# ebu/libear

Hardware: AMD Instinct MI355X
Metric: Msamples/s (higher is better)
Workload: dtype f32 io / f16x2-split MFMA, f32 accumulate

## Files before the change

libear_amd/csrc/api_render.hip:

```cpp
#include <cmath>
#include <cstdlib>
#include <chrono>
#include <memory>
#include <vector>

#include "common.h"
#include "curves.h"
#include "host_pipeline.h"
#include "pcm_frames.h"
#include "fft_kernels.h"
#include "render_kernels.h"

using namespace earhip;

namespace earhip {
std::vector<cf> make_twiddles(int L) {
  std::vector<cf> tw(L);
  const double pi = 3.14159265358979323846264338327950288;
  for (int t = 0; t < L; t++) {
    const double a = -2.0 * pi * (double)t / (double)L;
    tw[t] = cf_make((float)std::cos(a), (float)std::sin(a));
  }
  return tw;
}

template <int L>
static void launch_spectrum_t(const float *in, size_t stride, int n_valid, const cf *tw, cf *out,
                              int rows, hipStream_t s) {
  hipLaunchKernelGGL((k_spectrum_real<L>), dim3(rows), dim3(kFftThreads), 0, s, in, stride,
                     n_valid, tw, out);
}
void launch_spectrum(int L, const float *in, size_t stride, int n_valid, const cf *tw, cf *out,
                     int rows, hipStream_t s) {
  switch (L) {
    case 64: launch_spectrum_t<64>(in, stride, n_valid, tw, out, rows, s); break;
    case 128: launch_spectrum_t<128>(in, stride, n_valid, tw, out, rows, s); break;
    case 256: launch_spectrum_t<256>(in, stride, n_valid, tw, out, rows, s); break;
    case 512: launch_spectrum_t<512>(in, stride, n_valid, tw, out, rows, s); break;
    case 1024: launch_spectrum_t<1024>(in, stride, n_valid, tw, out, rows, s); break;
    case 2048: launch_spectrum_t<2048>(in, stride, n_valid, tw, out, rows, s); break;
    case 4096: launch_spectrum_t<4096>(in, stride, n_valid, tw, out, rows, s); break;
    case 8192: launch_spectrum_t<8192>(in, stride, n_valid, tw, out, rows, s); break;
    default: {
      FftShape S;
      if (!fft_make_shape(L, &S)) fail_invalid("FFT size must be in [4, 8192]");
      hipLaunchKernelGGL(k_spectrum_real_rt, dim3(rows), dim3(kFftThreads), fft_rt_lds(k_spectrum_real_rt, L), s, S,
                         in, stride, n_valid, tw, out);
    }
  }
  EARHIP_HIP(hipGetLastError());
}
}

template <int L>
static void launch_decor_t(const DecorParams &P, dim3 grid, hipStream_t s) {
  hipLaunchKernelGGL((k_decorrelate_delay_mix<L>), grid, dim3(256), 0, s, P);
}
static void launch_decor(int L, const DecorParams &P, dim3 grid, hipStream_t s, bool force_wg) {
  switch (L) {
    case 128: launch_decor_t<128>(P, grid, s); break;
    case 256: launch_decor_t<256>(P, grid, s); break;
    case 512: launch_decor_t<512>(P, grid, s); break;
    case 1024:
      if (force_wg) {
        launch_decor_t<1024>(P, grid, s);
      } else {
        hipLaunchKernelGGL(k_decorrelate_wave, dim3((grid.x + kDecorWaves - 1) / kDecorWaves, grid.y),
                           dim3(64 * kDecorWaves), 0, s, P);
      }
      break;
    case 2048: launch_decor_t<2048>(P, grid, s); break;
    case 4096: launch_decor_t<4096>(P, grid, s); break;
    case 8192: launch_decor_t<8192>(P, grid, s); break;
    default: {
      FftShape S;
      if (!fft_make_shape(L, &S)) fail_invalid("block_size must be in [16, 4096]");
      const size_t lds = fft_rt_lds(k_decorrelate_delay_mix_rt, L, sizeof(float) * (L / 2));
      hipLaunchKernelGGL(k_decorrelate_delay_mix_rt, grid, dim3(256), lds, s, P, S);
    }
  }
  EARHIP_HIP(hipGetLastError());
}

static int wave_run_len(int T, int N, int num_cus) {
  const double c[4] = {0.0, 6.9, 9.3, 12.2};
  int best = 1;
  double best_cost = 1e30;
  for (int R = 1; R <= 31; R += 2) {
    const long runs = (T + R - 1) / R;
    const long wgs = (runs + earhip::kDecorWaves - 1) / earhip::kDecorWaves * N;
    const long full = wgs / (3L * num_cus), rem = wgs - full * 3L * num_cus;
    const double pairs = (R + 1) / 2;
    const double cost = pairs * (full * c[3] + c[(rem + num_cus - 1) / num_cus]);
    if (cost <= best_cost) best_cost = cost, best = R;
    if (runs == 1) break;
  }
  return best;
}

struct earhip_render {
  earhip_ctx *ctx = nullptr;
  int M = 0, N = 0, B = 0, K = 1, D = 0, T = 0;
  int Bk = 0, Lk = 0;
  int NP = 1;
  std::unique_ptr<CurveSet> curves;
  int64_t t = 0;
  int last_plan[3] = {0, 0, 0};
  int last_paired = -1;
  size_t last_scratch_bytes = 0;
  long scratch_regrows = 0;
  DevBuf<unsigned> rec;
  bool last_gated = false;
  bool last_device_form = false;
  bool last_hg_robust = false;
  int last_kind = -1;
  int run_len = 11;
  bool run_len_set = false;

  DevBuf<SegDesc> desc;
  DevBuf<float> bus;
  int max_gsplit = 1;
  DevBuf<cf> H, tw;
  DevBuf<float> tail[2], dly[2], hist[2];
  DevBuf<float> ztail, zdly, zhist;
  bool fresh = true;
  int cur = 0;
  DevBuf<float> d_in, d_out;
  PinBuf<float> p_in, p_out;
  std::unique_ptr<GatherPool> gather;
  StreamPipe pipe;
  int last_host_chunks = 0;
  PinBuf<unsigned char> p_bytes;
  DevBuf<unsigned char> d_bytes;
  DevBuf<float> d_ilv, d_rows, d_rows_out;
  DevBuf<unsigned char> d_pcm;
  PinBuf<unsigned char> p_pcm;
  PcmLevels levels;
  bool timing = false;
  bool last_timed = false;
  int timing_every = 1;
  long timing_calls = 0;
  hipEvent_t ev[6] = {nullptr, nullptr, nullptr, nullptr, nullptr, nullptr};
  struct Pending { hipEvent_t e[6]; bool has_k2; bool continues; };
  std::vector<Pending> pending;
  std::vector<hipEvent_t> pool;
  double acc_ms[3] = {0, 0, 0};
  double acc_n[3] = {0, 0, 0};

  ~earhip_render() {
    for (auto &p : pending)
      for (auto e : p.e)
        if (e) (void)hipEventDestroy(e);
    for (auto e : pool) (void)hipEventDestroy(e);
  }

  unsigned mode_word() {
    ctx->use();
    unsigned word = 0;
    EARHIP_HIP(hipMemcpyAsync(&word, rec.p, sizeof(word), hipMemcpyDeviceToHost, ctx->stream));
    EARHIP_HIP(hipStreamSynchronize(ctx->stream));
    if (!(word & kModeRecorded)) fail_internal("no gain kernel recorded the call's mode word");
    return word;
  }

  hipEvent_t get_event() {
    if (!pool.empty()) {
      hipEvent_t e = pool.back();
      pool.pop_back();
      return e;
    }
    hipEvent_t e;
    EARHIP_HIP(hipEventCreate(&e));
    return e;
  }

  void drain_timing() {
    EARHIP_HIP(hipStreamSynchronize(ctx->stream));
    for (auto &p : pending) {
      float ms = 0;
      const double one = p.continues ? 0.0 : 1.0;
      EARHIP_HIP(hipEventElapsedTime(&ms, p.e[0], p.e[1]));
      acc_ms[2] += ms; acc_n[2] += one;
      EARHIP_HIP(hipEventElapsedTime(&ms, p.e[2], p.e[3]));
      acc_ms[0] += ms; acc_n[0] += one;
      if (p.has_k2) {
        EARHIP_HIP(hipEventElapsedTime(&ms, p.e[4], p.e[5]));
        acc_ms[1] += ms; acc_n[1] += one;
      }
      for (auto e : p.e)
        if (e) pool.push_back(e);
    }
    pending.clear();
  }

  size_t direct_stride(const float *const *ch, int count, size_t n) const {
    if (ctx->host_ranges.empty() || count < 1) return 0;
    const uintptr_t a0 = (uintptr_t)ch[0];
    const uintptr_t step = count > 1 ? (uintptr_t)ch[1] - a0 : sizeof(float) * n;
    if ((a0 & 15) != 0 || step % 16 != 0 || step < sizeof(float) * n || step > ((uintptr_t)1 << 40)) return 0;
    for (int c = 1; c < count; c++)
      if ((uintptr_t)ch[c] - (uintptr_t)ch[c - 1] != step) return 0;
    return ctx->host_reachable(ch[0], step * (count - 1) + sizeof(float) * n) ? (size_t)(step / sizeof(float)) : 0;
  }

  size_t frames_to_device_rows(size_t nblocks, const void *frames_dev, int fmt, int frame_channels, int first_channel, bool with_out) {
    ctx->use();
    const size_t S = (size_t)pcm_sample_bytes(fmt), n = nblocks * (size_t)B, cap = (size_t)T * B;
    if (d_rows.n < cap * M || (with_out && d_rows_out.n < cap * N)) {
      EARHIP_HIP(hipStreamSynchronize(ctx->stream));
      d_rows.reserve(cap * M);
      if (with_out) d_rows_out.reserve(cap * N);
    }
    launch_pcm_to_rows(fmt, frames_dev, (size_t)frame_channels * S, (size_t)first_channel * S, M, n, d_rows.p, n, ctx->stream);
    return n;
  }
  void reserve_pcm_out(size_t bytes, bool pinned) {
    levels.reserve(N, ctx->stream);
    d_pcm.reserve(bytes);
    if (pinned) p_pcm.reserve(bytes);
  }

  HostChunkPlan host_plan(size_t nblocks, bool direct) const {
    return plan_host_chunks(nblocks, B, M, direct, ctx->has(OPT_HOST_CHUNK_MB), ctx->get(OPT_HOST_CHUNK_MB), ctx->get(OPT_HOST_FIRST, 0));
  }
  hipError_t chunk_rows_d2h(float *out0, size_t out_st, size_t at, size_t len) {
    const float *dout = d_out.p + (size_t)N * at;
    if (out_st)
      return hipMemcpy2DAsync(out0 + at, sizeof(float) * out_st, dout, sizeof(float) * len, sizeof(float) * len, N, hipMemcpyDeviceToHost, pipe.out);
    return hipMemcpyAsync(p_out.p + (size_t)N * at, dout, sizeof(float) * len * N, hipMemcpyDeviceToHost, pipe.out);
  }
  void chunk_rows_scatter(float *const *out, size_t at, size_t len) const {
    for (int ch = 0; ch < N; ch++) std::memcpy(out[ch] + at, p_out.p + (size_t)N * at + (size_t)ch * len, sizeof(float) * len);
  }
  void process_short_call(size_t nblocks, float *out0, size_t out_st) {
    const size_t n = nblocks * (size_t)B;
    const bool direct_out = NP <= 1;
    process_device(nblocks, d_in.p, n, out_st ? out0 : direct_out ? p_out.p : d_out.p, out_st ? out_st : n);
    if (!out_st && !direct_out) EARHIP_HIP(hipMemcpyAsync(p_out.p, d_out.p, sizeof(float) * n * N, hipMemcpyDeviceToHost, ctx->stream));
  }
  GatherPool &staging_threads() {
    if (!gather) {
      gather.reset(new GatherPool);
      const int want = ctx->get(OPT_HOST_THREADS, 0);
      gather->start(want >= 1 && want <= 64 ? want : default_staging_threads());
    }
    return *gather;
  }

  MixLaunch plan_call(size_t nblocks, size_t in_stride) {
    const int nsamples = (int)(nblocks * (size_t)B);
    MixLaunch ml = plan_mix(ctx, curves->plan(), M, nsamples, ctx->strict, max_gsplit, curves->aligned_tile(t),
                            curves->ramp_share(), curves->gain_scale(), curves->point_density_all(), curves->pair_waste(256), curves->pair_waste(512),
                            curves->hinge_exact_share(in_stride, (size_t)nsamples), curves->tiles_aligned(kF32GridTile, t),
                            curves->deltas_per_pair(256));
    const size_t bus_stride = ((size_t)nsamples + 3) & ~(size_t)3;
    while (ml.gsplit > 1 && bus_stride * K * N * ml.gsplit > bus.n) ml.gsplit /= 2;
    return ml;
  }

  size_t last_in_stride = 0;
  void reserve_for_curves() {
    size_t need = 0;
    bool hinge = false;
    const size_t lens[3] = {(size_t)T, (size_t)std::max(1, T / 2), (size_t)1};
    for (size_t nb : lens) {
      const MixLaunch ml = plan_call(nb, last_in_stride ? last_in_stride : nb * (size_t)B);
      need = std::max(need, scratch_units(*curves, ml, M));
      hinge = hinge || ml.hinge;
    }
    if (hinge) curves->ensure_kinks(ctx);
// ... 3 lines not shown
    }
  }

  int resident_workgroups(const MixLaunch &ml) const {
    if (!(ml.split || ml.pieces || ml.hinge)) return 0;
    return ctx->num_cus * (ml.tile() >= 512 ? 1 : 2);
  }

  struct BusTap {
    float *sink = nullptr;
    size_t stride = 0, cap = 0, pos = 0;
    void attach(bool on, float *sink_dev, size_t sink_stride, size_t sink_capacity) {
      if (on) {
        require(sink_dev != nullptr, "sink_dev must not be NULL");
        require(sink_stride >= sink_capacity, "sink_stride must be >= sink_capacity");
      }
      *this = on ? BusTap{sink_dev, sink_stride, sink_capacity, 0} : BusTap{};
    }
  };
  earhip_loudness *meter = nullptr;
  earhip_firmix *fm = nullptr;
  earhip_limiter *lim = nullptr;
  BusTap fm_tap, lim_tap;
  void check_taps(size_t nblocks) const {
    const size_t n = nblocks * (size_t)B;
    if (meter) loudness_check_room(meter, n);
    if (fm) {
      firmix_check_room(fm, nblocks);
      if (fm_tap.pos + n > fm_tap.cap) fail_invalid("the call would pass the FIR matrix's sink_capacity (nothing was rendered)");
    }
    if (lim) {
      limiter_check_room(lim, n);
      if (lim_tap.pos + n > lim_tap.cap) fail_invalid("the call would pass the limiter's sink_capacity (nothing was rendered)");
    }
  }
  void feed_taps(size_t nblocks, const float *out_dev, size_t out_stride) {
    const size_t n = nblocks * (size_t)B;
    if (meter) loudness_feed(meter, n, out_dev, out_stride);
    if (fm) {
      firmix_feed(fm, nblocks, out_dev, out_stride, fm_tap.sink + fm_tap.pos, fm_tap.stride);
      fm_tap.pos += n;
    }
    if (lim) {
      limiter_feed(lim, n, out_dev, out_stride, lim_tap.sink + lim_tap.pos, lim_tap.stride);
      lim_tap.pos += n;
    }
  }
  void process_device(size_t nblocks, const float *in_dev, size_t in_stride, float *out_dev, size_t out_stride) {
    if (!meter && !fm && !lim) return render_spans(nblocks, in_dev, in_stride, out_dev, out_stride);
    check_taps(nblocks);
    render_spans(nblocks, in_dev, in_stride, out_dev, out_stride);
    feed_taps(nblocks, out_dev, out_stride);
  }
  void render_spans(size_t nblocks, const float *in_dev, size_t in_stride, float *out_dev, size_t out_stride) {
    MixLaunch whole;
    bool have_plan = false;
    if (!ctx->strict && ctx->get(OPT_TAILCUT, 1) != 0 && nblocks >= 2) {
      last_in_stride = in_stride;
      if (curves->dirty()) {
        curves->commit(ctx);
        reserve_for_curves();
      }
      const MixLaunch ml = whole = plan_call(nblocks, in_stride);
      have_plan = true;
      const int W = resident_workgroups(ml);
      if (W > 0 && ml.gsplit == 1 && ml.ntiles > W) {
        const size_t tile = (size_t)ml.tile();
        const size_t full = (size_t)ml.ntiles / (size_t)W, rest = (size_t)ml.ntiles % (size_t)W;
        const size_t main_samples = full * (size_t)W * tile;
        const size_t eighths = (size_t)std::min(std::max(ctx->get(OPT_TAILCUT, 2), 0), 7);
        if (rest > 0 && rest <= (size_t)W * eighths / 8 && main_samples % (size_t)B == 0) {
          const size_t main_blocks = main_samples / (size_t)B;
          process_span(main_blocks, in_dev, in_stride, out_dev, out_stride, false);
          const int kind = last_kind, plan3[3] = {last_plan[0], last_plan[1], last_plan[2]};
          const size_t scratch = last_scratch_bytes;
          const bool gated = last_gated, device_form = last_device_form, hg_robust = last_hg_robust;
          const int paired = last_paired;
          process_span(nblocks - main_blocks, in_dev + main_samples, in_stride, out_dev + main_samples, out_stride, true);
          last_kind = kind;
          last_gated = gated, last_device_form = device_form, last_paired = paired, last_hg_robust = hg_robust;
          for (int i = 0; i < 3; i++) last_plan[i] = plan3[i];
          last_scratch_bytes = scratch;
          last_tail_blocks = (int)(nblocks - main_blocks);
          return;
        }
      }
    }
    last_tail_blocks = 0;
    process_span(nblocks, in_dev, in_stride, out_dev, out_stride, false, have_plan ? &whole : nullptr);
  }
  int last_tail_blocks = 0;

  void process_span(size_t nblocks, const float *in_dev, size_t in_stride, float *out_dev,
                    size_t out_stride, bool continues, const MixLaunch *planned = nullptr) {
    const int nsamples = (int)(nblocks * (size_t)B);
    last_in_stride = in_stride;
    if (curves->dirty()) {
      curves->commit(ctx);
      reserve_for_curves();
    }
    const bool strict = ctx->strict;
    MixLaunch ml = planned ? *planned : plan_call(nblocks, in_stride);
    if (ml.hinge) curves->ensure_kinks(ctx);

    last_kind = ml.f32grid ? 2 : ml.hinge ? 5 : ml.pieces ? 4 : ml.split ? 3 : ml.mfma ? 1 : 0;
    {
      const size_t need = scratch_units(*curves, ml, M);
      if (need > desc.n) {
        EARHIP_HIP(hipStreamSynchronize(ctx->stream));
        desc.reserve(need + need / 2);
        scratch_regrows++;
      }
      last_scratch_bytes = need * 16;
    }
    const size_t bus_stride = ((size_t)nsamples + 3) & ~(size_t)3;
    const size_t part_stride = bus_stride * K * N;
    if (part_stride * ml.gsplit > bus.n) fail_internal("bus buffer too small for this launch plan");
    last_paired = (ml.pieces || ml.hinge) ? (ml.paired ? 1 : 0) : -1;
    last_plan[0] = ml.tile();
    last_plan[1] = ml.ntiles;
    last_plan[2] = ml.gsplit;
    Pending pd;
    hipEvent_t *evp = nullptr;
    const bool timed = timing && (continues ? last_timed : (timing_calls++ % timing_every) == 0);
    last_timed = timed;
    if (timed) {
      for (int i = 0; i < 6; i++) pd.e[i] = get_event();
      pd.has_k2 = K == 2;
      pd.continues = continues;
      evp = pd.e;
    }
    const long lazy_before = ctx->lazy_allocs;
    ctx->record_slot = rec.p + (continues ? 1 : 0);
    if (K == 1) {
      if (ml.gsplit == 1) {
        launch_gain_mix(ctx, *curves, ml, strict, t, nsamples, in_dev, in_stride, out_dev,
                        out_stride, 0, desc.p, evp);
      } else {
        launch_gain_mix(ctx, *curves, ml, strict, t, nsamples, in_dev, in_stride, bus.p,
                        bus_stride, part_stride, desc.p, evp);
        hipLaunchKernelGGL(k_sum_parts, dim3((nsamples + 255) / 256, N), dim3(256), 0,
                           ctx->stream, bus.p, part_stride, ml.gsplit, bus_stride, N, nsamples,
                           out_dev, out_stride);
        EARHIP_HIP(hipGetLastError());
      }
    } else {
      launch_gain_mix(ctx, *curves, ml, strict, t, nsamples, in_dev, in_stride, bus.p,
                      bus_stride, part_stride, desc.p, evp);
      DecorParams P;
      P.bus = bus.p;
      P.bus_stride = bus_stride;
      P.part_stride = part_stride;
      P.nparts = ml.gsplit;
      const bool wave_k2 = Lk == 1024 && NP == 1 && !ctx->get(OPT_K2_WG);
      const int kblocks = (int)(nblocks * (size_t)(B / Bk));
      if (wave_k2 && ml.gsplit > 1) {
        if (evp) EARHIP_HIP(hipEventRecord(evp[4], ctx->stream));
        hipLaunchKernelGGL(k_sum_parts, dim3((nsamples + 255) / 256, K * N), dim3(256), 0, ctx->stream, bus.p,
                           part_stride, ml.gsplit, bus_stride, K * N, nsamples, bus.p, bus_stride);
        EARHIP_HIP(hipGetLastError());
        P.nparts = 1;
      }
      P.out = out_dev;
      P.out_stride = out_stride;
      P.tw = tw.p;
      P.dly_in = fresh ? zdly.p : dly[cur].p;
      P.dly_out = dly[cur ^ 1].p;
      P.N = N;
      P.T = kblocks;
      const int R = wave_k2 && !run_len_set ? wave_run_len(kblocks, N, ctx->num_cus) : run_len;
      P.R = R;
      P.D = D;
      P.hist_len = (NP - 1) * Bk;
      P.hist_in = fresh ? zhist.p : hist[cur].p;
      P.hist_out = hist[cur ^ 1].p;
      const dim3 grid((unsigned)((kblocks + R - 1) / R), N);
      if (evp && P.nparts == ml.gsplit) EARHIP_HIP(hipEventRecord(evp[4], ctx->stream));
      for (int part = 0; part < NP; part++) {
        P.H = H.p + (size_t)part * N * Lk;
        P.tail_in = (fresh ? ztail.p : tail[cur].p) + (fresh ? 0 : (size_t)part * N * Bk);
        P.tail_out = tail[cur ^ 1].p + (size_t)part * N * Bk;
        P.shift = part * Bk;
        P.accumulate = part > 0 ? 1 : 0;
        if (wave_k2) {
          hipLaunchKernelGGL(k_decorrelate_wave, dim3((grid.x + kDecorWaves - 1) / kDecorWaves, grid.y), dim3(64 * kDecorWaves),
                             0, ctx->stream, P);
          EARHIP_HIP(hipGetLastError());
        } else {
          launch_decor(Lk, P, grid, ctx->stream, true);
        }
      }
      if (evp) EARHIP_HIP(hipEventRecord(evp[5], ctx->stream));
      cur ^= 1;
      fresh = false;
    }
    if (timed) pending.push_back(pd);
    last_gated = ctx->last_gate_idx >= 0;
    last_device_form = ctx->last_wide_idx >= 0;
    last_hg_robust = last_gated && ctx->last_hinge_robust;
    if (ctx->lazy_allocs != lazy_before) scratch_regrows++;
    t += nsamples;
  }
};

extern "C" {

int earhip_render_create(earhip_ctx *ctx, const earhip_render_config *cfg, earhip_render **out) {
  return guarded([&] {
    require(ctx != nullptr && cfg != nullptr && out != nullptr, "NULL argument");
    require(cfg->n_objects >= 1 && cfg->n_out >= 1, "n_objects and n_out must be >= 1");
    require(cfg->n_buses == 1 || cfg->n_buses == 2, "n_buses must be 1 or 2");
    FftShape shape;
    require(cfg->block_size >= 16 && cfg->block_size <= 4096 && fft_make_shape(2 * cfg->block_size, &shape),
            "block_size must be in [16, 4096]");
    require(cfg->max_blocks >= 1, "max_blocks must be >= 1");
    require((int64_t)cfg->max_blocks * cfg->block_size < ((int64_t)1 << 30),
            "max_blocks * block_size too large");
    require(cfg->delay >= 0, "delay must be >= 0");
    if (cfg->n_buses == 2) {
      require(cfg->decorrelators != nullptr && cfg->n_taps >= 1,
              "n_buses == 2 needs decorrelator filters");
      require((cfg->n_taps + cfg->block_size - 1) / cfg->block_size <= 64,
              "decorrelator filters of more than 64 blocks are not supported by the fused render "
              "(use BlockConvolver)");
    } else {
      require(cfg->delay == 0, "delay needs n_buses == 2");
    }
    ctx->use();
    std::unique_ptr<earhip_render> r(new earhip_render);
    r->ctx = ctx;
    r->M = cfg->n_objects;
    r->N = cfg->n_out;
    r->B = cfg->block_size;
    r->K = cfg->n_buses;
    r->D = cfg->delay;
    r->T = cfg->max_blocks;
    r->Bk = r->B;
    if (r->K == 2 && r->B > 512 && r->B % 512 == 0 && cfg->n_taps <= 512 && !ctx->get(OPT_K2_OWN_BLOCK)) r->Bk = 512;
    r->Lk = 2 * r->Bk;
    if (r->Lk == 2048) r->run_len = 7;
    if (ctx->has(OPT_RUN)) {
      const int v = ctx->get(OPT_RUN);
      if (v >= 1 && v <= 255) r->run_len = v | 1, r->run_len_set = true;
    }
    r->curves.reset(new CurveSet(r->M, r->K * r->N, r->K, false));
    const size_t max_samples = (size_t)r->T * r->B;
    reserve_call_words(ctx, r->M, max_samples);
    r->rec.alloc_zero(2, ctx->stream);
    const size_t min_tile = (size_t)std::min(16 * ctx->nrt, std::min(64 * ctx->spl, 256));
    const size_t max_tiles = (max_samples + min_tile - 1) / min_tile;
    r->desc.alloc((size_t)r->M * ((max_samples + 255) / 256) + 1);
    (void)max_tiles;
    r->max_gsplit = 16;
    if (ctx->has(OPT_GSPLIT)) {
      const int v = ctx->get(OPT_GSPLIT);
      if (v >= 1 && v <= 32) r->max_gsplit = v;
    }
    r->bus.alloc_zero((size_t)r->K * r->N * bus_samples_bound(ctx, max_samples, r->max_gsplit), ctx->stream);
    if (r->K == 2) {
      const auto tw = make_twiddles(r->Lk);
      r->tw.alloc(r->Lk);
      EARHIP_HIP(hipMemcpy(r->tw.p, tw.data(), sizeof(cf) * r->Lk, hipMemcpyHostToDevice));
      r->NP = (cfg->n_taps + r->Bk - 1) / r->Bk;
      const size_t rows = (size_t)r->NP * r->N;
      std::vector<float> parts(rows * r->Bk, 0.0f);
      for (int n = 0; n < r->N; n++)
        for (int t = 0; t < cfg->n_taps; t++)
          parts[((size_t)(t / r->Bk) * r->N + n) * r->Bk + t % r->Bk] = cfg->decorrelators[(size_t)n * cfg->n_taps + t];
      DevBuf<float> taps;
      taps.alloc(parts.size());
      EARHIP_HIP(hipMemcpy(taps.p, parts.data(), sizeof(float) * parts.size(), hipMemcpyHostToDevice));
      r->H.alloc(rows * r->Lk);
      launch_spectrum(r->Lk, taps.p, r->Bk, r->Bk, r->tw.p, r->H.p, (int)rows, ctx->stream);
      EARHIP_HIP(hipStreamSynchronize(ctx->stream));
      std::vector<cf> h(rows * r->Lk);
      EARHIP_HIP(hipMemcpy(h.data(), r->H.p, sizeof(cf) * h.size(), hipMemcpyDeviceToHost));
      for (size_t n = 0; n < rows; n++) {
        cf *hn = h.data() + n * r->Lk;
        hn[0].y = 0.0f;
        hn[r->Bk].y = 0.0f;
        for (int k = 1; k < r->Bk; k++) hn[r->Lk - k] = cf_conj(hn[k]);
      }
      EARHIP_HIP(hipMemcpy(r->H.p, h.data(), sizeof(cf) * h.size(), hipMemcpyHostToDevice));
      const size_t hist_n = (size_t)r->N * std::max((r->NP - 1) * r->Bk, 1);
      for (int i = 0; i < 2; i++) {
        r->tail[i].alloc_zero(rows * r->Bk, ctx->stream);
        r->dly[i].alloc_zero((size_t)r->N * std::max(r->D, 1), ctx->stream);
        r->hist[i].alloc_zero(hist_n, ctx->stream);
        if (i == 0) {
          r->ztail.alloc_zero((size_t)r->N * r->Bk, ctx->stream);
          r->zdly.alloc_zero((size_t)r->N * std::max(r->D, 1), ctx->stream);
          r->zhist.alloc_zero(hist_n, ctx->stream);
        }
      }
    }
    EARHIP_HIP(hipStreamSynchronize(ctx->stream));
    *out = r.release();
  });
}

int earhip_render_destroy(earhip_render *r) {
  return guarded([&] {
    if (!r) return;
    (void)hipSetDevice(r->ctx->device);
    (void)hipStreamSynchronize(r->ctx->stream);
    delete r;
  });
}

int earhip_render_set_object_points(earhip_render *r, int object, int npoints,
                                    const int64_t *times, const float *direct,
                                    const float *diffuse) {
  return guarded([&] {
    require(r != nullptr, "render must not be NULL");
    require(npoints >= 1, "interp_points must not be empty");
    require(times != nullptr && direct != nullptr, "times/direct must not be NULL");
    require(r->K == 1 || diffuse != nullptr, "diffuse gains must not be NULL when n_buses == 2");
    const int N = r->N, cols = r->K * N;
    std::vector<float> rows((size_t)npoints * cols);
    for (int k = 0; k < npoints; k++) {
      std::memcpy(&rows[(size_t)k * cols], direct + (size_t)k * N, sizeof(float) * N);
      if (r->K == 2)
        std::memcpy(&rows[(size_t)k * cols + N], diffuse + (size_t)k * N, sizeof(float) * N);
    }
    r->curves->set_object(object, npoints, times, rows.data());
  });
}

int earhip_render_commit(earhip_render *r) {
  return guarded([&] {
    require(r != nullptr, "render must not be NULL");
    r->ctx->use();
    r->curves->commit(r->ctx);
    r->reserve_for_curves();
  });
}

int earhip_render_reset(earhip_render *r, int64_t sample_time) {
  return guarded([&] {
    require(r != nullptr, "render must not be NULL");
    r->ctx->use();
    r->t = sample_time;
    r->fresh = true;
    r->levels.zero(r->ctx->stream);
  });
}

int earhip_render_attach_loudness(earhip_render *r, earhip_loudness *m) {
  return guarded([&] {
    require(r != nullptr, "render must not be NULL");
    if (m) {
      require(loudness_ctx(m) == r->ctx, "the meter must belong to the renderer's context");
      require(loudness_channels(m) == r->N, "the meter must have n_out channels");
    }
    r->meter = m;
  });
}

int earhip_render_attach_firmix(earhip_render *r, earhip_firmix *fm, float *sink_dev, size_t sink_stride, size_t sink_capacity) {
  return guarded([&] {
    require(r != nullptr, "render must not be NULL");
    if (fm) {
      require(firmix_ctx(fm) == r->ctx, "the FIR matrix must belong to the renderer's context");
      require(firmix_inputs(fm) == r->N, "the FIR matrix must have n_in = the renderer's n_out");
      require(firmix_block(fm) == r->B, "the FIR matrix must have the renderer's block size");
    }
    r->fm_tap.attach(fm != nullptr, sink_dev, sink_stride, sink_capacity);
    r->fm = fm;
  });
}

int earhip_render_firmix_position(earhip_render *r, size_t *samples) {
  return guarded([&] {
    require(r != nullptr && samples != nullptr, "render and samples must not be NULL");
    *samples = r->fm_tap.pos;
  });
}

int earhip_render_attach_limiter(earhip_render *r, earhip_limiter *lim, float *sink_dev, size_t sink_stride, size_t sink_capacity) {
  return guarded([&] {
    require(r != nullptr, "render must not be NULL");
    if (lim) {
      require(limiter_ctx(lim) == r->ctx, "the limiter must belong to the renderer's context");
      require(limiter_channels(lim) == r->N, "the limiter must have n_channels = the renderer's n_out");
    }
    r->lim_tap.attach(lim != nullptr, sink_dev, sink_stride, sink_capacity);
    r->lim = lim;
  });
}

int earhip_render_limiter_position(earhip_render *r, size_t *samples) {
  return guarded([&] {
    require(r != nullptr && samples != nullptr, "render and samples must not be NULL");
    *samples = r->lim_tap.pos;
  });
}

int earhip_render_process_device(earhip_render *r, size_t nblocks, const float *in_dev,
                                 size_t in_stride, float *out_dev, size_t out_stride) {
  return guarded([&] {
    require(r != nullptr, "render must not be NULL");
    require(in_dev != nullptr && out_dev != nullptr, "device pointers must not be NULL");
    require(nblocks <= (size_t)r->T, "nblocks exceeds max_blocks");
    r->check_taps(nblocks);
    require(in_stride >= nblocks * r->B && out_stride >= nblocks * r->B, "stride too small");
    if (nblocks == 0) return;
    r->ctx->use();
    r->process_device(nblocks, in_dev, in_stride, out_dev, out_stride);
  });
}

int earhip_render_process(earhip_render *r, size_t nblocks, const float *const *in,
                          float *const *out) {
  return guarded([&] {
    require(r != nullptr, "render must not be NULL");
    require(in != nullptr && out != nullptr, "in and out must not be NULL");
    require(nblocks <= (size_t)r->T, "nblocks exceeds max_blocks");
    r->check_taps(nblocks);
    if (nblocks == 0) return;
    earhip_ctx *ctx = r->ctx;
    ctx->use();
    const size_t n = nblocks * r->B;
    const size_t cap = (size_t)r->T * r->B;
    r->p_in.reserve(cap * r->M);
    r->p_out.reserve(cap * r->N);
    r->d_in.reserve(cap * r->M);
    r->d_out.reserve(cap * r->N);
    const bool dbg = ctx->get(OPT_DEBUG_TIMING) != 0;
    auto now = [] { return std::chrono::duration<double, std::micro>(std::chrono::steady_clock::now().time_since_epoch()).count(); };
    const double t_a = dbg ? now() : 0.0;
    const bool short_call = r->host_plan(nblocks, false).short_call;
    const size_t in_st = r->direct_stride(in, r->M, n);
    const size_t out_st = r->NP <= 1 || !short_call ? r->direct_stride(out, r->N, n) : 0;
    r->last_host_chunks = 0;
    if (!short_call) {
      const HostChunkPlan plan = r->host_plan(nblocks, in_st != 0);
      r->pipe.make();
// ... 334 lines not shown
```

libear_amd/csrc/render_kernels.h:

```cpp
#pragma once

#include <hip/hip_runtime.h>

#include "fft_lds.h"

namespace earhip {

struct DecorParams {
  const float *bus;
  size_t bus_stride;
  size_t part_stride;
  int nparts;
  float *out;
  size_t out_stride;
  const cf *H;
  const cf *tw;
  const float *tail_in;
  float *tail_out;
  const float *dly_in;
  float *dly_out;
  int N, T, R, D;
  int shift = 0;
  int accumulate = 0;
  int hist_len = 0;
// ... 494 lines not shown
  d = DIR < 0 ? wave_add_i(a1, t) : wave_sub_i(a1, t);
}
template <int DIR, bool TA>
__device__ __forceinline__ void wave_r4_tw(v2f &a, v2f &b, v2f &c, v2f &d, v2f wa, v2f wb, v2f wc, v2f wd) {
  const v2f pa = TA ? wave_cmul<DIR>(a, wa) : a;
  const v2f a0 = wave_cmul_acc<DIR>(c, wc, pa), a1 = wave_twice_minus(pa, a0);
  const v2f pb = wave_cmul<DIR>(b, wb);
  const v2f a2 = wave_cmul_acc<DIR>(d, wd, pb), t = wave_twice_minus(pb, a2);
  wave_r4_out<DIR>(a0, a1, a2, t, a, b, c, d);
}
template <int DIR, bool HALF, bool STAGE1>
__device__ __forceinline__ void wave_dft16_f(v2f (&v)[16]) {
  const float c1 = 0.92387953251128674f, s1 = 0.38268343236508977f, r2 = 0.70710678118654752f;
  if (STAGE1) {
#pragma unroll
    for (int n2 = 0; n2 < 4; n2++) {
      if (HALF) {
        const v2f a = v[n2], b = v[n2 + 4];
        v[n2] = a + b;
        v[n2 + 8] = a - b;
        v[n2 + 4] = DIR < 0 ? wave_sub_i(a, b) : wave_add_i(a, b);
        v[n2 + 12] = DIR < 0 ? wave_add_i(a, b) : wave_sub_i(a, b);
      } else {
        wave_r4<DIR>(v[n2], v[n2 + 4], v[n2 + 8], v[n2 + 12]);
      }
    }
  }
  const v2f W1 = {c1, -s1}, W3 = {s1, -c1}, W9 = {-c1, s1}, R2 = {r2, r2};
  wave_r4<DIR>(v[0], v[1], v[2], v[3]);
  {
    const v2f u = DIR < 0 ? wave_sub_i(v[6], v[6]) : wave_add_i(v[6], v[6]);
    const v2f a0 = wave_fma_k(u, R2, v[4]), a1 = wave_fnma_k(u, R2, v[4]);
    const v2f pb = wave_cmul_k<DIR>(v[5], W1);
    const v2f a2 = wave_cmul_acc_k<DIR>(v[7], W3, pb), t = wave_twice_minus(pb, a2);
    wave_r4_out<DIR>(a0, a1, a2, t, v[4], v[5], v[6], v[7]);
  }
  {
    const v2f u9 = DIR < 0 ? wave_sub_i(v[9], v[9]) : wave_add_i(v[9], v[9]);
    const v2f u11 = DIR < 0 ? wave_add_i(v[11], v[11]) : wave_sub_i(v[11], v[11]);
    const v2f a0 = DIR < 0 ? wave_sub_i(v[8], v[10]) : wave_add_i(v[8], v[10]);
    const v2f a1 = DIR < 0 ? wave_add_i(v[8], v[10]) : wave_sub_i(v[8], v[10]);
    const v2f sm = u9 - u11, q = u9 + u11;
    v[8] = wave_fma_k(sm, R2, a0);
    v[10] = wave_fnma_k(sm, R2, a0);
    v[9] = DIR < 0 ? wave_fma_k_subi(q, R2, a1) : wave_fma_k_addi(q, R2, a1);
    v[11] = DIR < 0 ? wave_fma_k_addi(q, R2, a1) : wave_fma_k_subi(q, R2, a1);
  }
  {
    const v2f u = DIR < 0 ? wave_add_i(v[14], v[14]) : wave_sub_i(v[14], v[14]);
    const v2f a0 = wave_fnma_k(u, R2, v[12]), a1 = wave_fma_k(u, R2, v[12]);
    const v2f pb = wave_cmul_k<DIR>(v[13], W3);
    const v2f a2 = wave_cmul_acc_k<DIR>(v[15], W9, pb), t = wave_twice_minus(pb, a2);
    wave_r4_out<DIR>(a0, a1, a2, t, v[12], v[13], v[14], v[15]);
  }
  v2f t;
#define EARHIP_SW(a, b) t = v[a], v[a] = v[b], v[b] = t;
  EARHIP_SW(1, 4) EARHIP_SW(2, 8) EARHIP_SW(3, 12) EARHIP_SW(6, 9) EARHIP_SW(7, 13) EARHIP_SW(11, 14)
#undef EARHIP_SW
}

__device__ __forceinline__ int wave_pad(int i) { return i + (i >> 4); }

template <int DIR, bool HALF = false>
__device__ __forceinline__ void wave_fft1024(v2f (&v)[16], v2f *lds, const v2f *t1, const v2f *t2, int lane) {
#if EARHIP_K2_FOLDED
  wave_dft16_f<DIR, HALF, true>(v);
#pragma unroll
  for (int r = 0; r < 16; r++) lds[wave_pad(16 * lane + r)] = v[r];
#pragma unroll
  for (int r = 0; r < 16; r++) v[r] = lds[wave_pad(lane + 64 * r)];
  __builtin_amdgcn_sched_barrier(0);
  wave_r4_tw<DIR, false>(v[0], v[4], v[8], v[12], v[0], t1[3], t1[7], t1[11]);
  __builtin_amdgcn_sched_barrier(0);
#pragma unroll
  for (int n2 = 1; n2 < 4; n2++) {
    wave_r4_tw<DIR, true>(v[n2], v[n2 + 4], v[n2 + 8], v[n2 + 12], t1[n2 - 1], t1[n2 + 3], t1[n2 + 7], t1[n2 + 11]);
    __builtin_amdgcn_sched_barrier(0);
  }
  wave_dft16_f<DIR, false, false>(v);
  __builtin_amdgcn_sched_barrier(0);
  const int ob = (lane >> 4) * 256 + (lane & 15);
#pragma unroll
  for (int r = 0; r < 16; r++) lds[wave_pad(ob + 16 * r)] = v[r];
#pragma unroll
  for (int q = 0; q < 4; q++)
#pragma unroll
    for (int r = 0; r < 4; r++) v[q + 4 * r] = lds[wave_pad(lane + 64 * q + 256 * r)];
  __builtin_amdgcn_sched_barrier(0);
#pragma unroll
  for (int q = 0; q < 4; q++) {
    const int j = lane + 64 * q;
    wave_r4_tw<DIR, false>(v[q], v[q + 4], v[q + 8], v[q + 12], v[q], t2[j], t2[256 + j], t2[512 + j]);
    __builtin_amdgcn_sched_barrier(0);
  }
#else
  wave_dft16<DIR>(v);
#pragma unroll
  for (int r = 0; r < 16; r++) lds[wave_pad(16 * lane + r)] = v[r];
#pragma unroll
  for (int r = 0; r < 16; r++) v[r] = lds[wave_pad(lane + 64 * r)];
  __builtin_amdgcn_sched_barrier(0);
#pragma unroll
  for (int r = 1; r < 16; r++) {
    v[r] = wave_cmul<DIR>(v[r], t1[r - 1]);
    if ((r & 3) == 3) __builtin_amdgcn_sched_barrier(0);
  }
  wave_dft16<DIR>(v);
  __builtin_amdgcn_sched_barrier(0);
  const int ob = (lane >> 4) * 256 + (lane & 15);
#pragma unroll
  for (int r = 0; r < 16; r++) lds[wave_pad(ob + 16 * r)] = v[r];
#pragma unroll
  for (int q = 0; q < 4; q++)
#pragma unroll
    for (int r = 0; r < 4; r++) v[q + 4 * r] = lds[wave_pad(lane + 64 * q + 256 * r)];
  __builtin_amdgcn_sched_barrier(0);
#pragma unroll
  for (int q = 0; q < 4; q++) {
#pragma unroll
    for (int r = 1; r < 4; r++) v[q + 4 * r] = wave_cmul<DIR>(v[q + 4 * r], t2[256 * (r - 1) + lane + 64 * q]);
    wave_r4<DIR>(v[q], v[q + 4], v[q + 8], v[q + 12]);
    __builtin_amdgcn_sched_barrier(0);
  }
#endif
}

constexpr int kDecorWaves = 4;

#ifdef EARHIP_K2_PROF
static __device__ unsigned long long g_k2_prof[2][32];
#define EARHIP_K2_MARK(i)                                                                        \
  do {                                                                                           \
    if (prof_slot >= 0 && lane == 0 && (i) < 32) g_k2_prof[prof_slot][(i)] = __builtin_readcyclecounter(); \
  } while (0)
#else
#define EARHIP_K2_MARK(i) do {} while (0)
#endif

__global__ void __launch_bounds__(64 * kDecorWaves) __attribute__((amdgpu_waves_per_eu(3, 3))) k_decorrelate_wave(DecorParams P) {
  constexpr int L = 1024, B = 512;
  __shared__ v2f lds_all[kDecorWaves][L + L / 16];
  __shared__ v2f h_lds[L + L / 16];
  __shared__ v2f t1_lds[16][17];
  __shared__ v2f t2_lds[3 * 256];
  const int lane = threadIdx.x & 63, w = __builtin_amdgcn_readfirstlane(threadIdx.x >> 6);
  v2f *lds = lds_all[w];
  auto to_v2f = [](cf c) { return v2f{c.x, c.y}; };
  const int n = blockIdx.y;
#ifdef EARHIP_K2_PROF
  const int prof_slot = w != 0 ? -1 : (blockIdx.x == 0 && blockIdx.y == 0) ? 0 : (blockIdx.x == gridDim.x / 2 && blockIdx.y == gridDim.y / 2) ? 1 : -1;
  int prof_i = 2;
#endif
  EARHIP_K2_MARK(0);
  for (int i = threadIdx.x; i < L; i += 64 * kDecorWaves) h_lds[wave_pad(i)] = to_v2f(P.H[(size_t)n * L + i]);
  if (threadIdx.x < 240) {
    const int k = threadIdx.x / 15, r = threadIdx.x % 15 + 1;
    t1_lds[k][r - 1] = to_v2f(P.tw[(4 * r * k) & (L - 1)]);
  }
  for (int i = threadIdx.x; i < 3 * 256; i += 64 * kDecorWaves) t2_lds[i] = to_v2f(P.tw[((i >> 8) + 1) * (i & 255)]);
  __syncthreads();
  EARHIP_K2_MARK(1);
  const int first = (blockIdx.x * kDecorWaves + w) * P.R;
  if (first >= P.T) return;
  const int last = min(first + P.R, P.T);
  const float norm = 1.0f / (float)(2 * B);
  const float *direct = P.bus + (size_t)n * P.bus_stride;
  const float *diffuse = P.bus + (size_t)(P.N + n) * P.bus_stride;
  float *out = P.out + (size_t)n * P.out_stride;

  const v2f *t1 = t1_lds[lane & 15];
  const v2f *t2 = t2_lds;

  auto bus_at = [&](const float *row, int s) {
    const float *q = row + s;
    float v = q[0];
    for (int p = 1; p < P.nparts; p++) v += q[(size_t)p * P.part_stride];
    return v;
  };
  auto bus_at8 = [&](const float *row, int s0, float (&acc)[8]) {
    const float *q = row + s0 + lane;
#if EARHIP_K2_ABL >= 2
#pragma unroll
    for (int m = 0; m < 8; m++) acc[m] = (float)(lane - m) * 1e-3f;
    return;
#endif
#pragma unroll
    for (int m = 0; m < 8; m++) acc[m] = __builtin_nontemporal_load(q + 64 * m);
    for (int p = 1; p < P.nparts; p++) {
      q += P.part_stride;
#pragma unroll
      for (int m = 0; m < 8; m++) acc[m] += __builtin_nontemporal_load(q + 64 * m);
    }
  };
  auto delayed = [&](int s) {
    const int sd = s - P.D;
    return sd >= 0 ? bus_at(direct, sd) : P.dly_in[(size_t)n * P.D + (sd + P.D)];
  };
  auto delayed8 = [&](int tb, float (&acc)[8]) {
    if (tb * B >= P.D) {
      bus_at8(direct, tb * B - P.D, acc);
    } else {
      const int s0 = tb * B - P.D + lane;
      const float *q = direct + s0;
#pragma unroll
      for (int m = 0; m < 8; m++)
        acc[m] = s0 + 64 * m < 0 ? P.dly_in[(size_t)n * P.D + (s0 + 64 * m + P.D)] : q[64 * m];
      for (int p = 1; p < P.nparts; p++) {
        q += P.part_stride;
#pragma unroll
        for (int m = 0; m < 8; m++)
          if (s0 + 64 * m >= 0) acc[m] += q[64 * m];
      }
    }
  };

  float tl[8];
#pragma unroll
  for (int m = 0; m < 8; m++) tl[m] = first == 0 ? P.tail_in[(size_t)n * B + lane + 64 * m] : 0.0f;

  auto load_half = [&](int tb, v2f (&z)[8], auto im_tag) {
    constexpr bool IM = decltype(im_tag)::value;
    const float *q = diffuse + tb * B + lane;
#pragma unroll
    for (int m = 0; m < 8; m++) {
#if EARHIP_K2_ABL >= 2
      const float x = (float)(lane + m) * 1e-3f;
#else
      const float x = __builtin_nontemporal_load(q + 64 * m);
#endif
      if (IM) z[m].y = x;
      else z[m].x = x;
    }
    for (int p = 1; p < P.nparts; p++) {
      q += P.part_stride;
#pragma unroll
      for (int m = 0; m < 8; m++) {
        const float x = __builtin_nontemporal_load(q + 64 * m);
        if (IM) z[m].y += x;
        else z[m].x += x;
      }
    }
  };
  auto load_pair = [&](int tb, v2f (&z)[8]) {
#pragma unroll
    for (int m = 0; m < 8; m++) z[m] = v2f{0.0f, 0.0f};
    if (tb >= 0 && tb < last) load_half(tb, z, std::false_type{});
    if (tb + 1 < last) load_half(tb + 1, z, std::true_type{});
  };
  v2f v[16];
  {
    v2f z[8];
    load_pair(first - 1, z);
#pragma unroll
    for (int m = 0; m < 8; m++) v[m] = z[m];
  }
  for (int tb = first - 1; tb < last; tb += 2) {
    const bool have_re = tb >= 0, have_im = tb + 1 < last;
#pragma unroll
    for (int m = 0; m < 8; m++) v[m + 8] = v2f{0.0f, 0.0f};
    v2f z[8];
    load_pair(tb + 2, z);
    float dre[8], dim[8];
#pragma unroll
    for (int m = 0; m < 8; m++) dre[m] = dim[m] = 0.0f;
    if (have_re && tb >= first) delayed8(tb, dre);
    if (have_im) delayed8(tb + 1, dim);
#ifdef EARHIP_K2_PROF
    EARHIP_K2_MARK(prof_i);
    asm volatile("s_waitcnt vmcnt(0)" ::: "memory");
    EARHIP_K2_MARK(prof_i + 1);
#endif
    wave_fft1024<-1, true>(v, lds, t1, t2, lane);
#ifdef EARHIP_K2_PROF
    asm volatile("" : "+v"(v[0]));
    EARHIP_K2_MARK(prof_i + 2);
#endif
#pragma unroll
    for (int m = 0; m < 16; m++) {
      v[m] = wave_cmul<-1>(v[m], h_lds[wave_pad(lane + 64 * m)]);
      if ((m & 3) == 3) __builtin_amdgcn_sched_barrier(0);
    }
#ifdef EARHIP_K2_PROF
    asm volatile("" : "+v"(v[0]));
    EARHIP_K2_MARK(prof_i + 3);
#endif
    wave_fft1024<+1>(v, lds, t1, t2, lane);
#ifdef EARHIP_K2_PROF
    asm volatile("" : "+v"(v[0]));
    EARHIP_K2_MARK(prof_i + 4);
    prof_i += 5;
#endif
#pragma unroll
    for (int m = 0; m < 8; m++) {
      dre[m] = (v[m].x + tl[m]) * norm + dre[m];
      asm volatile("" : "+v"(dre[m]) : : "memory");
      tl[m] = have_re ? v[m + 8].x : tl[m];
    }
#pragma unroll
    for (int m = 0; m < 8; m++) {
      dim[m] = (v[m].y + tl[m]) * norm + dim[m];
      asm volatile("" : "+v"(dim[m]) : : "memory");
      tl[m] = have_im ? v[m + 8].y : tl[m];
    }
#pragma unroll
    for (int m = 0; m < 8; m++) {
      v[m] = z[m];
      asm volatile("" : "+v"(v[m]) : : "memory");
    }
    __builtin_amdgcn_sched_barrier(0);
#if EARHIP_K2_ABL == 1 || EARHIP_K2_ABL == 3
    if (have_im && dre[0] + dim[0] + dre[7] + dim[7] == 123.456f) out[tb * B + lane] = dre[1] + dim[1];
#else
    if (have_re && tb >= first) {
#pragma unroll
      for (int m = 0; m < 8; m++) __builtin_nontemporal_store(dre[m], out + tb * B + lane + 64 * m);
    }
    if (have_im) {
#pragma unroll
      for (int m = 0; m < 8; m++) __builtin_nontemporal_store(dim[m], out + (tb + 1) * B + lane + 64 * m);
    }
#endif
  }
  EARHIP_K2_MARK(prof_i < 31 ? prof_i : 31);
  if (last == P.T) {
#pragma unroll
    for (int m = 0; m < 8; m++) P.tail_out[(size_t)n * B + lane + 64 * m] = tl[m];
    const int total = P.T * B;
    if (total >= P.D && P.D <= 256) {
      const float *q = direct + (total - P.D) + lane;
      float acc[4] = {0.0f, 0.0f, 0.0f, 0.0f};
      bool ok[4];
#pragma unroll
      for (int k = 0; k < 4; k++) ok[k] = lane + 64 * k < P.D;
      int p = 0;
      for (; p + 3 < P.nparts; p += 4) {
        float t[4][4];
#pragma unroll
        for (int j = 0; j < 4; j++)
#pragma unroll
          for (int k = 0; k < 4; k++) t[j][k] = ok[k] ? q[(size_t)(p + j) * P.part_stride + 64 * k] : 0.0f;
#pragma unroll
        for (int k = 0; k < 4; k++) {
          acc[k] = p == 0 ? t[0][k] : acc[k] + t[0][k];
          acc[k] += t[1][k];
          acc[k] += t[2][k];
          acc[k] += t[3][k];
        }
      }
      for (; p < P.nparts; p++)
#pragma unroll
        for (int k = 0; k < 4; k++) {
          const float v = ok[k] ? q[(size_t)p * P.part_stride + 64 * k] : 0.0f;
          acc[k] = p == 0 ? v : acc[k] + v;
        }
#pragma unroll
      for (int k = 0; k < 4; k++)
        if (ok[k]) P.dly_out[(size_t)n * P.D + lane + 64 * k] = acc[k];
    } else {
      for (int j = lane; j < P.D; j += 64) P.dly_out[(size_t)n * P.D + j] = delayed(total + j);
    }
  }
}


}
```

Measured before the change: 1.121 million.

## Switch K2 wave decorrelator to overlap-save with balanced persistent wave partitioning

The 1024-point wave decorrelation kernel moves from overlap-add, which carries an output tail between blocks, to overlap-save. Each FFT input now pairs the previous input block with the current one, so the wrap-around half of the output is simply discarded. The wave run length is no longer picked from a cost model. Instead the grid is sized to fill the CUs (about 3 workgroups per CU across channels), and each wave gets an evenly divided contiguous span of block pairs. Initial loads of the previous block and the first pair are issued before the LDS twiddle/filter setup and barrier, so their latency overlaps the setup. The carry state moves from the tail buffer to the history buffer, whose allocation size changes to match. The first pair no longer needs the special-cased leading FFT, at the cost of re-reading one previous block per wave from memory.

```diff
diff --git a/libear_amd/csrc/api_render.hip b/libear_amd/csrc/api_render.hip
--- a/libear_amd/csrc/api_render.hip
+++ b/libear_amd/csrc/api_render.hip
@@ -65,8 +65,7 @@
       if (force_wg) {
         launch_decor_t<1024>(P, grid, s);
       } else {
-        hipLaunchKernelGGL(k_decorrelate_wave, dim3((grid.x + kDecorWaves - 1) / kDecorWaves, grid.y),
-                           dim3(64 * kDecorWaves), 0, s, P);
+        hipLaunchKernelGGL(k_decorrelate_wave, grid, dim3(64 * kDecorWaves), 0, s, P);
       }
       break;
     case 2048: launch_decor_t<2048>(P, grid, s); break;
@@ -82,20 +81,10 @@
   EARHIP_HIP(hipGetLastError());
 }
 
-static int wave_run_len(int T, int N, int num_cus) {
-  const double c[4] = {0.0, 6.9, 9.3, 12.2};
-  int best = 1;
-  double best_cost = 1e30;
-  for (int R = 1; R <= 31; R += 2) {
-    const long runs = (T + R - 1) / R;
-    const long wgs = (runs + earhip::kDecorWaves - 1) / earhip::kDecorWaves * N;
-    const long full = wgs / (3L * num_cus), rem = wgs - full * 3L * num_cus;
-    const double pairs = (R + 1) / 2;
-    const double cost = pairs * (full * c[3] + c[(rem + num_cus - 1) / num_cus]);
-    if (cost <= best_cost) best_cost = cost, best = R;
-    if (runs == 1) break;
-  }
-  return best;
+static int wave_groups(int T, int N, int num_cus) {
+  const int pairs = (T + 1) / 2;
+  const int fit = std::max(1, 3 * num_cus / N);
+  return std::min(fit, (pairs + earhip::kDecorWaves - 1) / earhip::kDecorWaves);
 }
 
 struct earhip_render {
@@ -115,7 +104,8 @@
   bool last_hg_robust = false;
   int last_kind = -1;
   int run_len = 11;
-  bool run_len_set = false;
+  int wave_run = 0;
+  bool wave_k2 = false;
 
   DevBuf<SegDesc> desc;
   DevBuf<float> bus;
@@ -425,7 +415,7 @@
       P.bus_stride = bus_stride;
       P.part_stride = part_stride;
       P.nparts = ml.gsplit;
-      const bool wave_k2 = Lk == 1024 && NP == 1 && !ctx->get(OPT_K2_WG);
+      if (fresh) wave_k2 = Lk == 1024 && NP == 1 && !ctx->get(OPT_K2_WG);
       const int kblocks = (int)(nblocks * (size_t)(B / Bk));
       if (wave_k2 && ml.gsplit > 1) {
         if (evp) EARHIP_HIP(hipEventRecord(evp[4], ctx->stream));
@@ -441,13 +431,14 @@
       P.dly_out = dly[cur ^ 1].p;
       P.N = N;
       P.T = kblocks;
-      const int R = wave_k2 && !run_len_set ? wave_run_len(kblocks, N, ctx->num_cus) : run_len;
+      const int R = wave_k2 ? wave_run : run_len;
       P.R = R;
       P.D = D;
       P.hist_len = (NP - 1) * Bk;
       P.hist_in = fresh ? zhist.p : hist[cur].p;
       P.hist_out = hist[cur ^ 1].p;
-      const dim3 grid((unsigned)((kblocks + R - 1) / R), N);
+      const dim3 grid(wave_k2 ? (unsigned)(R > 0 ? ((kblocks + R - 1) / R + kDecorWaves - 1) / kDecorWaves : wave_groups(kblocks, N, ctx->num_cus))
+                              : (unsigned)((kblocks + R - 1) / R), N);
       if (evp && P.nparts == ml.gsplit) EARHIP_HIP(hipEventRecord(evp[4], ctx->stream));
       for (int part = 0; part < NP; part++) {
         P.H = H.p + (size_t)part * N * Lk;
@@ -456,8 +447,7 @@
         P.shift = part * Bk;
         P.accumulate = part > 0 ? 1 : 0;
         if (wave_k2) {
-          hipLaunchKernelGGL(k_decorrelate_wave, dim3((grid.x + kDecorWaves - 1) / kDecorWaves, grid.y), dim3(64 * kDecorWaves),
-                             0, ctx->stream, P);
+          hipLaunchKernelGGL(k_decorrelate_wave, grid, dim3(64 * kDecorWaves), 0, ctx->stream, P);
           EARHIP_HIP(hipGetLastError());
         } else {
           launch_decor(Lk, P, grid, ctx->stream, true);
@@ -514,7 +504,7 @@
     if (r->Lk == 2048) r->run_len = 7;
     if (ctx->has(OPT_RUN)) {
       const int v = ctx->get(OPT_RUN);
-      if (v >= 1 && v <= 255) r->run_len = v | 1, r->run_len_set = true;
+      if (v >= 1 && v <= 255) r->run_len = v | 1, r->wave_run = v;
     }
     r->curves.reset(new CurveSet(r->M, r->K * r->N, r->K, false));
     const size_t max_samples = (size_t)r->T * r->B;
@@ -555,7 +545,7 @@
         for (int k = 1; k < r->Bk; k++) hn[r->Lk - k] = cf_conj(hn[k]);
       }
       EARHIP_HIP(hipMemcpy(r->H.p, h.data(), sizeof(cf) * h.size(), hipMemcpyHostToDevice));
-      const size_t hist_n = (size_t)r->N * std::max((r->NP - 1) * r->Bk, 1);
+      const size_t hist_n = (size_t)r->N * std::max(r->NP - 1, 1) * r->Bk;
       for (int i = 0; i < 2; i++) {
         r->tail[i].alloc_zero(rows * r->Bk, ctx->stream);
         r->dly[i].alloc_zero((size_t)r->N * std::max(r->D, 1), ctx->stream);
diff --git a/libear_amd/csrc/render_kernels.h b/libear_amd/csrc/render_kernels.h
--- a/libear_amd/csrc/render_kernels.h
+++ b/libear_amd/csrc/render_kernels.h
@@ -670,24 +670,23 @@
   int prof_i = 2;
 #endif
   EARHIP_K2_MARK(0);
-  for (int i = threadIdx.x; i < L; i += 64 * kDecorWaves) h_lds[wave_pad(i)] = to_v2f(P.H[(size_t)n * L + i]);
-  if (threadIdx.x < 240) {
-    const int k = threadIdx.x / 15, r = threadIdx.x % 15 + 1;
-    t1_lds[k][r - 1] = to_v2f(P.tw[(4 * r * k) & (L - 1)]);
-  }
-  for (int i = threadIdx.x; i < 3 * 256; i += 64 * kDecorWaves) t2_lds[i] = to_v2f(P.tw[((i >> 8) + 1) * (i & 255)]);
-  __syncthreads();
-  EARHIP_K2_MARK(1);
-  const int first = (blockIdx.x * kDecorWaves + w) * P.R;
-  if (first >= P.T) return;
-  const int last = min(first + P.R, P.T);
+  int first, last;
+  {
+    const int wi = blockIdx.x * kDecorWaves + w;
+    if (P.R > 0) {
+      first = wi < (P.T + P.R - 1) / P.R ? wi * P.R : P.T;
+      last = min(first + P.R, P.T);
+    } else {
+      const unsigned pairs = (unsigned)(P.T + 1) / 2, waves = gridDim.x * kDecorWaves, q = pairs / waves, r = pairs - q * waves;
+      const unsigned p0 = wi * q + min((unsigned)wi, r), p1 = p0 + q + ((unsigned)wi < r ? 1u : 0u);
+      first = min((int)(2 * p0), P.T);
+      last = min((int)(2 * p1), P.T);
+    }
+  }
   const float norm = 1.0f / (float)(2 * B);
   const float *direct = P.bus + (size_t)n * P.bus_stride;
   const float *diffuse = P.bus + (size_t)(P.N + n) * P.bus_stride;
   float *out = P.out + (size_t)n * P.out_stride;
-
-  const v2f *t1 = t1_lds[lane & 15];
-  const v2f *t2 = t2_lds;
 
   auto bus_at = [&](const float *row, int s) {
     const float *q = row + s;
@@ -732,10 +731,6 @@
     }
   };
 
-  float tl[8];
-#pragma unroll
-  for (int m = 0; m < 8; m++) tl[m] = first == 0 ? P.tail_in[(size_t)n * B + lane + 64 * m] : 0.0f;
-
   auto load_half = [&](int tb, v2f (&z)[8], auto im_tag) {
     constexpr bool IM = decltype(im_tag)::value;
     const float *q = diffuse + tb * B + lane;
@@ -762,33 +757,60 @@
   auto load_pair = [&](int tb, v2f (&z)[8]) {
 #pragma unroll
     for (int m = 0; m < 8; m++) z[m] = v2f{0.0f, 0.0f};
-    if (tb >= 0 && tb < last) load_half(tb, z, std::false_type{});
+    if (tb < last) load_half(tb, z, std::false_type{});
     if (tb + 1 < last) load_half(tb + 1, z, std::true_type{});
   };
   v2f v[16];
-  {
-    v2f z[8];
-    load_pair(first - 1, z);
-#pragma unroll
-    for (int m = 0; m < 8; m++) v[m] = z[m];
-  }
-  for (int tb = first - 1; tb < last; tb += 2) {
-    const bool have_re = tb >= 0, have_im = tb + 1 < last;
-#pragma unroll
-    for (int m = 0; m < 8; m++) v[m + 8] = v2f{0.0f, 0.0f};
+  float cb[8];
+  auto take_pair = [&](int tb, const v2f (&z)[8]) {
+    const bool have_re = tb < last, have_im = tb + 1 < last;
+#pragma unroll
+    for (int m = 0; m < 8; m++) {
+      v[m] = v2f{cb[m], z[m].x};
+      v[m + 8] = z[m];
+      cb[m] = have_im ? z[m].y : have_re ? z[m].x : cb[m];
+      asm volatile("" : "+v"(v[m]), "+v"(v[m + 8]), "+v"(cb[m]) : : "memory");
+    }
+  };
+
+  v2f z0[8];
+  if (first < last) {
+    if (first == 0) {
+#pragma unroll
+      for (int m = 0; m < 8; m++) cb[m] = P.hist_in[(size_t)n * B + lane + 64 * m];
+    } else {
+      bus_at8(diffuse, (first - 1) * B, cb);
+    }
+    load_pair(first, z0);
+  }
+  for (int i = threadIdx.x; i < L; i += 64 * kDecorWaves) h_lds[wave_pad(i)] = to_v2f(P.H[(size_t)n * L + i]);
+  if (threadIdx.x < 240) {
+    const int k = threadIdx.x / 15, r = threadIdx.x % 15 + 1;
+    t1_lds[k][r - 1] = to_v2f(P.tw[(4 * r * k) & (L - 1)]);
+  }
+  for (int i = threadIdx.x; i < 3 * 256; i += 64 * kDecorWaves) t2_lds[i] = to_v2f(P.tw[((i >> 8) + 1) * (i & 255)]);
+  __syncthreads();
+  EARHIP_K2_MARK(1);
+  if (first >= last) return;
+  const v2f *t1 = t1_lds[lane & 15];
+  const v2f *t2 = t2_lds;
+  take_pair(first, z0);
+
+  for (int tb = first; tb < last; tb += 2) {
+    const bool have_im = tb + 1 < last;
     v2f z[8];
     load_pair(tb + 2, z);
     float dre[8], dim[8];
 #pragma unroll
-    for (int m = 0; m < 8; m++) dre[m] = dim[m] = 0.0f;
-    if (have_re && tb >= first) delayed8(tb, dre);
+    for (int m = 0; m < 8; m++) dim[m] = 0.0f;
+    delayed8(tb, dre);
     if (have_im) delayed8(tb + 1, dim);
 #ifdef EARHIP_K2_PROF
     EARHIP_K2_MARK(prof_i);
     asm volatile("s_waitcnt vmcnt(0)" ::: "memory");
     EARHIP_K2_MARK(prof_i + 1);
 #endif
-    wave_fft1024<-1, true>(v, lds, t1, t2, lane);
+    wave_fft1024<-1>(v, lds, t1, t2, lane);
 #ifdef EARHIP_K2_PROF
     asm volatile("" : "+v"(v[0]));
     EARHIP_K2_MARK(prof_i + 2);
@@ -810,29 +832,21 @@
 #endif
 #pragma unroll
     for (int m = 0; m < 8; m++) {
-      dre[m] = (v[m].x + tl[m]) * norm + dre[m];
+      dre[m] = v[m + 8].x * norm + dre[m];
       asm volatile("" : "+v"(dre[m]) : : "memory");
-      tl[m] = have_re ? v[m + 8].x : tl[m];
     }
 #pragma unroll
     for (int m = 0; m < 8; m++) {
-      dim[m] = (v[m].y + tl[m]) * norm + dim[m];
+      dim[m] = v[m + 8].y * norm + dim[m];
       asm volatile("" : "+v"(dim[m]) : : "memory");
-      tl[m] = have_im ? v[m + 8].y : tl[m];
-    }
-#pragma unroll
-    for (int m = 0; m < 8; m++) {
-      v[m] = z[m];
-      asm volatile("" : "+v"(v[m]) : : "memory");
-    }
+    }
+    take_pair(tb + 2, z);
     __builtin_amdgcn_sched_barrier(0);
 #if EARHIP_K2_ABL == 1 || EARHIP_K2_ABL == 3
     if (have_im && dre[0] + dim[0] + dre[7] + dim[7] == 123.456f) out[tb * B + lane] = dre[1] + dim[1];
 #else
-    if (have_re && tb >= first) {
-#pragma unroll
-      for (int m = 0; m < 8; m++) __builtin_nontemporal_store(dre[m], out + tb * B + lane + 64 * m);
-    }
+#pragma unroll
+    for (int m = 0; m < 8; m++) __builtin_nontemporal_store(dre[m], out + tb * B + lane + 64 * m);
     if (have_im) {
 #pragma unroll
       for (int m = 0; m < 8; m++) __builtin_nontemporal_store(dim[m], out + (tb + 1) * B + lane + 64 * m);
@@ -842,7 +856,7 @@
   EARHIP_K2_MARK(prof_i < 31 ? prof_i : 31);
   if (last == P.T) {
 #pragma unroll
-    for (int m = 0; m < 8; m++) P.tail_out[(size_t)n * B + lane + 64 * m] = tl[m];
+    for (int m = 0; m < 8; m++) P.hist_out[(size_t)n * B + lane + 64 * m] = cb[m];
     const int total = P.T * B;
     if (total >= P.D && P.D <= 256) {
       const float *q = direct + (total - P.D) + lane;
```

Result: no change. 1.133 million, median of 2 (+1.1%).
